# shichaoy/cube_slam

Hardware: NVIDIA H100
Metric: scored cuboid proposals/s (higher is better)
Workload: dtype f64

## Files before the change

### cube_slam_b200/_lib.py

```python
import ctypes as C
import os
import sys

import numpy as np

_HERE = os.path.dirname(os.path.abspath(__file__))
LIB_PATH = os.path.join(_HERE, "lib", "libcubeslam_b200.so")

CS_OK = 0
STATUS_NAMES = {0: "CS_OK", -1: "CS_ERR_INVALID_ARG", -2: "CS_ERR_CUDA", -3: "CS_ERR_CAPACITY",
                -4: "CS_ERR_NOT_PREPARED", -5: "CS_ERR_NCCL", -6: "CS_ERR_UNSUPPORTED"}


class CuboidParams(C.Structure):
    _fields_ = [
        ("consider_config_1", C.c_int32), ("consider_config_2", C.c_int32),
        ("whether_sample_cam_roll_pitch", C.c_int32), ("whether_sample_bbox_height", C.c_int32),
        ("max_cuboid_num", C.c_int32), ("reweight_edge_distance", C.c_int32),
        ("whether_normalize_two_errors", C.c_int32), ("top_sample_count_override", C.c_int32),
        ("nominal_skew_ratio", C.c_double), ("max_cut_skew", C.c_double),
        ("vp12_edge_angle_thre", C.c_double), ("vp3_edge_angle_thre", C.c_double),
        ("shorted_edge_thre", C.c_double), ("weight_vp_angle", C.c_double), ("weight_skew_error", C.c_double),
        ("pre_merge_dist_thre", C.c_double), ("pre_merge_angle_thre", C.c_double),
        ("edge_length_threshold", C.c_double), ("canny_low", C.c_double), ("canny_high", C.c_double),
# ... 85 lines not shown
    d.data = int(cai["data"][0])
    d.n_frames, d.height, d.width = shape[:3]
    d.channels = shape[3] if len(shape) == 4 else 1
    d.stride_frame, d.stride_row, d.stride_col = strides[:3]
    d.stride_channel = strides[3] if len(shape) == 4 else 0
    if isinstance(order, str):
        if order.lower() not in ORDERS:
            raise ValueError("order must be 'bgr' or 'rgb', got %r" % order)
        order = ORDERS[order.lower()]
    d.channel_order = int(order)
    d.stream = _stream_handle(frames, stream) or None
    return d


_lib = None

EXPORTS = [
    "cs_abi_version", "cs_create", "cs_destroy", "cs_last_error", "cs_default_cuboid_params",
    "cs_default_line_params", "cs_set_calibration", "cs_cam_pose", "cs_cuboid_measurement", "cs_cuboid_measurement_orb", "cs_detect_cuboids", "cs_detect_cuboids_batch",
    "cs_batch_upload", "cs_batch_upload_online", "cs_detect_frames_batch", "cs_batch_run", "cs_batch_run_async", "cs_batch_fetch", "cs_batch_stats_get",
    "cs_batch_device_records", "cs_stream", "cs_stage_ms", "cs_set_profiling", "cs_debug_roi",
    "cs_debug_candidates", "cs_detect_lines", "cs_detect_lines_batch", "cs_debug_lsd", "cs_debug_lsd_stats", "cs_debug_lsd_prof", "cs_debug_atan2", "cs_atan2_host", "cs_cuboid_draw_edges", "cs_debug_edlines", "cs_debug_stage_offsets", "cs_comm_unique_id", "cs_comm_init",
    "cs_allgather_topk", "cs_allgather_wait", "cs_fetch_gathered",
    "cs_keylines_from_lines", "cs_lbd_compute", "cs_lbd_compute_batch", "cs_detect_descrip_lines", "cs_detect_descrip_lines_batch",
    "cs_match_line_descrip", "cs_match_line_descrip_batch", "cs_lbd_debug_prepare", "cs_lbd_debug_keylines_edl", "cs_debug_last_set_pose",
]
DEVICE_FRAME_EXPORTS = ["cs_check_device_frames", "cs_batch_upload_device", "cs_batch_upload_online_device", "cs_detect_lines_batch_device"]
EXPORTS += DEVICE_FRAME_EXPORTS
MATCHER_EXPORTS = ["cs_knn_match_line_descrip", "cs_knn_match_line_descrip_batch", "cs_radius_match_line_descrip", "cs_radius_match_line_descrip_batch"]
EXPORTS += MATCHER_EXPORTS
COLLECTION_EXPORTS = ["cs_lbd_collection_create", "cs_lbd_collection_destroy", "cs_lbd_collection_add", "cs_lbd_collection_clear",
                      "cs_lbd_collection_size", "cs_lbd_collection_match", "cs_lbd_collection_knn_match", "cs_lbd_collection_radius_match"]
EXPORTS += COLLECTION_EXPORTS
LSD_DEBUG_EXPORTS = ["cs_debug_lsd_defb", "cs_debug_lsd_occupancy"]
EXPORTS += LSD_DEBUG_EXPORTS
NFA_DEBUG_EXPORTS = ["cs_debug_nfa"]
EXPORTS += NFA_DEBUG_EXPORTS
LBD_DEVICE_FRAME_EXPORTS = ["cs_detect_descrip_lines_batch_device", "cs_lbd_compute_batch_device"]
EXPORTS += LBD_DEVICE_FRAME_EXPORTS
OCTAVE_EXPORTS = ["cs_detect_raw_lines_octaves_batch", "cs_detect_descrip_lines_octaves_batch", "cs_detect_raw_lines_octaves_batch_device",
                  "cs_detect_descrip_lines_octaves_batch_device"]
EXPORTS += OCTAVE_EXPORTS
LBD_OCTAVE_EXPORTS = ["cs_lbd_compute_octaves_batch", "cs_lbd_compute_octaves_batch_device"]
EXPORTS += LBD_OCTAVE_EXPORTS
MIXED_EXPORTS = ["cs_detect_lines_batch_mixed", "cs_detect_raw_lines_octaves_batch_mixed"]
EXPORTS += MIXED_EXPORTS


def load():
    global _lib
    if _lib is not None:
        return _lib
    if not os.path.exists(LIB_PATH):
        raise OSError("%s is missing: build it with `python -m cube_slam_b200.build` (needs nvcc); "
                      "cube_slam_b200 has no CPU fallback" % LIB_PATH)
    L = C.CDLL(LIB_PATH)
    vp, i, d_p = C.c_void_p, C.c_int, C.POINTER(C.c_double)
    u8_p, i32_p, f_p = C.POINTER(C.c_uint8), C.POINTER(C.c_int32), C.POINTER(C.c_float)
    L.cs_abi_version.restype = i
    L.cs_create.restype = vp
    L.cs_create.argtypes = [i] * 6
    L.cs_destroy.argtypes = [vp]
    L.cs_destroy.restype = None
    L.cs_last_error.restype = C.c_char_p
    L.cs_last_error.argtypes = [vp]
    L.cs_default_cuboid_params.argtypes = [C.POINTER(CuboidParams)]
    L.cs_default_line_params.argtypes = [C.POINTER(LineParams)]
    L.cs_set_calibration.argtypes = [vp, d_p]
    L.cs_cam_pose.argtypes = [d_p, d_p, d_p, d_p]
    L.cs_cuboid_measurement.argtypes = [vp, d_p, d_p, d_p, d_p, d_p, d_p, d_p]
    L.cs_cuboid_measurement_orb.argtypes = [vp, d_p, C.c_double, d_p, d_p, d_p, d_p]
    L.cs_detect_cuboids.argtypes = [vp, u8_p, i, i, i, i, d_p, d_p, i, d_p, i, C.POINTER(CuboidParams), vp, i32_p]
    L.cs_detect_cuboids_batch.argtypes = [vp, vp, i, i, i, i, i, d_p, d_p, i32_p, d_p, i32_p, C.POINTER(CuboidParams), vp, i32_p]
    L.cs_batch_upload.argtypes = [vp, vp, i, i, i, i, i, d_p, d_p, i32_p, d_p, i32_p, C.POINTER(CuboidParams)]
    L.cs_batch_upload_online.argtypes = [vp, vp, i, i, i, i, i, d_p, d_p, i32_p, C.POINTER(LineParams), C.POINTER(CuboidParams)]
    L.cs_detect_frames_batch.argtypes = [vp, vp, i, i, i, i, i, d_p, d_p, i32_p, C.POINTER(LineParams), C.POINTER(CuboidParams), vp, i32_p]
    L.cs_batch_run.argtypes = [vp]
    L.cs_batch_run_async.argtypes = [vp]
    L.cs_batch_fetch.argtypes = [vp, vp, i32_p]
    L.cs_batch_stats_get.argtypes = [vp, C.POINTER(BatchStats)]
    L.cs_batch_device_records.argtypes = [vp, C.POINTER(vp), C.POINTER(C.c_size_t)]
    L.cs_stream.restype = vp
    L.cs_stream.argtypes = [vp]
    L.cs_stage_ms.argtypes = [vp, C.c_char_p, C.POINTER(C.c_float)]
    L.cs_set_profiling.argtypes = [vp, i]
    L.cs_debug_stage_offsets.argtypes = [vp, vp, f_p]
    L.cs_debug_roi.argtypes = [vp, i, i32_p, u8_p, f_p, i, d_p, i, i32_p, i32_p]
    L.cs_debug_candidates.argtypes = [vp, i, i32_p, u8_p, d_p, d_p, i]
    L.cs_detect_lines.argtypes = [vp, vp, i, i, i, i, C.POINTER(LineParams), f_p, i32_p]
    L.cs_detect_lines_batch.argtypes = [vp, vp, i, i, i, i, i, C.POINTER(LineParams), f_p, C.c_int32, i32_p]
    L.cs_debug_lsd.argtypes = [vp, i, i32_p, d_p, d_p, d_p, i32_p, i32_p, f_p, i32_p, i]
    L.cs_debug_lsd_stats.argtypes = [vp, i32_p, i32_p, i]
    L.cs_debug_lsd_prof.argtypes = [vp, C.POINTER(C.c_uint64), i]
    if hasattr(L, "cs_debug_lsd_defb"):
        L.cs_debug_lsd_defb.argtypes = [vp, i, C.POINTER(C.c_uint32), i32_p]
    if hasattr(L, "cs_debug_lsd_occupancy"):
        L.cs_debug_lsd_occupancy.argtypes = [vp, i32_p]
    L.cs_debug_atan2.argtypes = [vp, d_p, d_p, d_p, i]
    L.cs_atan2_host.argtypes = [C.c_double, C.c_double]
    L.cs_atan2_host.restype = C.c_double
    if hasattr(L, "cs_debug_nfa"):
        L.cs_debug_nfa.argtypes = [vp, i32_p, i32_p, d_p, C.c_double, i, d_p, i32_p, i]
    L.cs_cuboid_draw_edges.argtypes = [vp, i32_p]
    L.cs_debug_edlines.argtypes = [vp, i, u8_p, C.POINTER(C.c_int16), C.POINTER(C.c_int16), C.POINTER(C.c_int16), u8_p, i32_p, i32_p, u8_p, f_p, i32_p, i]
    L.cs_comm_unique_id.argtypes = [vp, C.c_char_p, u8_p]
    L.cs_comm_init.argtypes = [vp, C.c_char_p, u8_p, i, i]
    L.cs_allgather_topk.argtypes = [vp, i, C.POINTER(vp)]
    L.cs_allgather_wait.argtypes = [vp]
    L.cs_fetch_gathered.argtypes = [vp, vp, i]
    L.cs_keylines_from_lines.argtypes = [f_p, i, i, i, vp]
    L.cs_lbd_compute.argtypes = [vp, vp, i, i, i, i, vp, i, u8_p, f_p]
    L.cs_lbd_compute_batch.argtypes = [vp, vp, i, i, i, i, i, vp, i32_p, u8_p, f_p]
    L.cs_detect_descrip_lines.argtypes = [vp, vp, i, i, i, i, C.POINTER(LineParams), vp, u8_p, i32_p]
    L.cs_detect_descrip_lines_batch.argtypes = [vp, vp, i, i, i, i, i, C.POINTER(LineParams), vp, u8_p, C.c_int32, i32_p]
    L.cs_match_line_descrip.argtypes = [vp, u8_p, i, u8_p, i, C.c_float, vp, i32_p]
    L.cs_match_line_descrip_batch.argtypes = [vp, u8_p, i32_p, u8_p, i32_p, i, C.c_float, vp, i32_p]
    i64_p = C.POINTER(C.c_int64)
    if all(hasattr(L, n) for n in MATCHER_EXPORTS):
        L.cs_knn_match_line_descrip.argtypes = [vp, u8_p, i, u8_p, i, i, u8_p, vp, i32_p]
        L.cs_knn_match_line_descrip_batch.argtypes = [vp, u8_p, i32_p, u8_p, i32_p, i, i, u8_p, vp, i32_p]
        L.cs_radius_match_line_descrip.argtypes = [vp, u8_p, i, u8_p, i, C.c_float, u8_p, vp, C.c_int64, i64_p]
        L.cs_radius_match_line_descrip_batch.argtypes = [vp, u8_p, i32_p, u8_p, i32_p, i, C.c_float, u8_p, vp, C.c_int64, i64_p]
    if all(hasattr(L, n) for n in COLLECTION_EXPORTS):
        L.cs_lbd_collection_create.restype = vp
        L.cs_lbd_collection_create.argtypes = [vp]
        L.cs_lbd_collection_destroy.restype = None
        L.cs_lbd_collection_destroy.argtypes = [vp]
        L.cs_lbd_collection_add.argtypes = [vp, u8_p, i32_p, i]
        L.cs_lbd_collection_clear.argtypes = [vp]
        L.cs_lbd_collection_size.argtypes = [vp, i32_p, i64_p]
# ... 43 lines not shown
```

### cube_slam_b200/csrc/cs_lsd.cu

```cuda
#include <cuda_runtime.h>
#include <float.h>
#include <math.h>
#include <stdint.h>

#include <algorithm>
#include <cmath>
#include <cstring>
#include <vector>

#include "cs_internal.h"
#include "cs_nfa.cuh"
#include "cs_tma.cuh"

#define LSD_PI 3.1415926535897932384626433832795
#define LSD_NOTDEF (-1024.0)
#define LSD_DEG2RAD (LSD_PI / 180)
#define LSD_3_2_PI ((3 * LSD_PI) / 2)
#define LSD_2PI (2 * LSD_PI)
#define LSD_LN10 2.30258509299404568402
#define LSD_NBINS 1024
#define LSD_CHUNK_ROWS 8
#define LSD_SCALE 0.8

#define LSD_CAND_CAP 2048
// ... 946 lines not shown
        ((sy < pre_boundary_thre) && (ey < pre_boundary_thre)) || ((sy > img_h - pre_boundary_thre) && (ey > img_h - pre_boundary_thre)))
        return false;
    const double ddx = (double)(e[0] - e[2]), ddy = (double)(e[1] - e[3]);
    const float line_length = (float)sqrt(ddx * ddx + ddy * ddy);
    if (!(line_length > line_length_thres)) return false;
    o[0] = sx;
    o[1] = sy;
    o[2] = ex;
    o[3] = ey;
    return true;
}

struct LsdGrowArgs {
    int W, H, img_w, img_h;
    uint4 *pix;
    const float *angf;
    const double *modgrad;
    int32_t *arena;
    int arena_cap;
    double LOG_NT;
    int min_reg_size;
    double prec, p, scale;
    float line_length_thres;
    float *raw;
    int32_t *n_raw;
    float *out;
    int32_t *n_out;
    int cap;
    LsdRect *cand;
    int32_t *n_cand;
    int cand_cap;
    int32_t *cand_line;
    struct LsdCandState *cand_state;
    int32_t *err;
    const double *lgam;
    uint32_t *ubits;
    const uint32_t *defb;
    const LsdGeom *geom;
};

template <bool kProf, bool kMixed>
__global__ void __launch_bounds__(32, 21) k_lsd_grow_seq(LsdGrowArgs A)
{
    const int f = blockIdx.x, lane = threadIdx.x;
    LsdGeom G = {};
    if constexpr (kMixed) G = A.geom[f];
    const int fW = kMixed ? G.W : A.W, fH = kMixed ? G.H : A.H;
    const size_t npx = (size_t)fW * fH;
    const size_t px0 = kMixed ? (size_t)G.px_off : f * npx;
    LsdFrame F;
    LSD_PROF_T0();
    F.W = fW;
    F.H = fH;
    F.pix = A.pix + px0;
    F.angf = A.angf + px0;
    F.modgrad = A.modgrad + px0;
    F.LOG_NT = kMixed ? G.LOG_NT : A.LOG_NT;
    const int WW = (fW + 31) >> 5, n_words = WW * fH;
    const size_t w0f = kMixed ? (size_t)G.bit_off : (size_t)f * n_words;
    F.ubits = A.ubits + w0f;
    F.WW = WW;
    F.span = nullptr;
    F.lgam = A.lgam;
    F.wmagic = ((1ull << 40) + (unsigned long long)fW - 1) / (unsigned long long)fW;
    for (int i = lane; i < n_words; i += 32) F.ubits[i] = 0u;
    __syncwarp();
// ... 23 lines not shown
            }
            if (!nz) break;
            const int j = __ffs(nz) - 1;
            const int b = __ffs(__shfl_sync(0xffffffffu, s, j)) - 1;
            const int s_addr = __shfl_sync(0xffffffffu, w_addr, j) + b;
            int n_all = 0, has_rect = 0;
            LsdRect rec;
            const long long c0 = kProf ? clock64() : 0ll;
            lsd_grow_candidate<kProf>(F, R, s_addr, min_reg_size, A.prec, A.p, n_all, has_rect, rec);
            if (kProf) {
                in_cand += clock64() - c0;
                if (lane == 0) {
                    atomicAdd(&g_lsd_prof[4], 1ull);
                    if (n_all > LSD_SEQ_SCAP) atomicAdd(&g_lsd_prof[8], 1ull);
                }
            }
            if (kProf) handoff_t0 = clock64();
            __syncwarp();
            u = wi < n_words ? __ldcg(F.ubits + wi) : 0u;
            u_next = wi + 32 < n_words ? __ldcg(F.ubits + wi + 32) : 0u;
            s = d & ~u & (lane > j ? 0xffffffffu : lane == j ? 0xfffffffeu << b : 0u);
            if (!has_rect) continue;
            const long long st0 = kProf ? clock64() : 0ll;
            if (lane == 0 && n_cand < A.cand_cap) A.cand[(size_t)f * A.cand_cap + n_cand] = rec;
            n_cand++;
            if (kProf) {
                const long long dt = clock64() - st0;
                if (lane == 0) atomicAdd(&g_lsd_prof[10], (unsigned long long)dt);
                handoff_t0 += dt;
            }
        }
    }
    if (kProf && lane == 0) atomicAdd(&g_lsd_prof[3], (unsigned long long)(clock64() - scan_t0 - in_cand));
    if (lane == 0) {
        A.n_cand[f] = n_cand;
        if (n_cand > A.cand_cap) {
            atomicOr(A.err, 4);
            atomicMax(A.err + 1, n_cand);
            A.err[2] = A.cand_cap;
        }
    }
    LSD_PROF_ADD(6);
}

#define LSD_VAL_CTAS 64

struct LsdCandState {
    double log_nfa;
    int32_t status;
    int32_t n;
    int32_t tot[5], alg[5];
};

__device__ int lsd_improve_variants(const LsdRect &rec, int round, LsdRect *cand)
{
    const double delta = 0.5, delta_2 = delta / 2.0;
    LsdRect r = rec;
    if (round == 0) {
        cand[0] = r;
        return 1;
    }
    if (round == 1) {
        for (int n = 0; n < 5; ++n) {
            r.p /= 2;
            r.prec = r.p * LSD_PI;
            cand[n] = r;
        }
        return 5;
    }
    const int phase = round - 2;
    int m = 0;
    for (int n = 0; n < 5; ++n)
        if ((r.width - delta) >= 0.5) {
            if (phase == 0)
                r.width -= delta;
            else if (phase == 1) {
                r.x1 += -r.dy * delta_2;
                r.y1 += r.dx * delta_2;
                r.x2 += -r.dy * delta_2;
                r.y2 += r.dx * delta_2;
                r.width -= delta;
            } else if (phase == 2) {
                r.x1 -= -r.dy * delta_2;
                r.y1 -= r.dx * delta_2;
                r.x2 -= -r.dy * delta_2;
                r.y2 -= r.dx * delta_2;
                r.width -= delta;
            } else {
                r.p /= 2;
                r.prec = r.p * LSD_PI;
            }
            cand[m++] = r;
        }
    return m;
}

template <bool kMixed>
__global__ void __launch_bounds__(128, 5) k_lsd_val_count(LsdGrowArgs A, int round)
{
    const int f = kMixed ? (int)(blockIdx.x / LSD_VAL_CTAS) : (int)blockIdx.y, lane = threadIdx.x & 31;
    const int bx = kMixed ? (int)(blockIdx.x % LSD_VAL_CTAS) : (int)blockIdx.x, gx = kMixed ? LSD_VAL_CTAS : (int)gridDim.x;
    LsdFrame F;
    if constexpr (kMixed) {
        const LsdGeom &G = A.geom[f];
        F.W = G.W;
        F.H = G.H;
        F.angf = A.angf + G.px_off;
        F.LOG_NT = G.LOG_NT;
    } else {
        const size_t npx = (size_t)A.W * A.H;
        F.W = A.W;
        F.H = A.H;
        F.angf = A.angf + f * npx;
        F.LOG_NT = A.LOG_NT;
    }
    F.pix = nullptr;
    F.modgrad = nullptr;
    F.ubits = nullptr;
    __shared__ LsdSpan s_span[4][5];
    F.span = s_span[threadIdx.x >> 5];
    F.lgam = A.lgam;
    F.wmagic = 0;
    const int n = min(A.n_cand[f], A.cand_cap);
    const int wpb = blockDim.x >> 5;
    for (int c = bx * wpb + (threadIdx.x >> 5); c < n; c += gx * wpb) {
        LsdCandState *S = A.cand_state + (size_t)f * A.cand_cap + c;
        if (round > 0 && S->status != 0) continue;
        const LsdRect rec = A.cand[(size_t)f * A.cand_cap + c];
        LsdRect cv[5];
        const int m = lsd_improve_variants(rec, round, cv);
        int tot[5] = {0, 0, 0, 0, 0}, alg[5] = {0, 0, 0, 0, 0};
        if (m == 1)
            lsd_rect_count(F, cv[0], tot[0], alg[0]);
        else if (m > 1)
            lsd_rect_count_multi(F, cv, m, round == 1 || round == 5, tot, alg);
        if (lane == 0) {
            S->n = m;
            for (int t = 0; t < 5; t++) {
                S->tot[t] = tot[t];
                S->alg[t] = alg[t];
            }
        }
    }
}

template <bool kMixed>
__global__ void __launch_bounds__(128, 5) k_lsd_val_nfa(LsdGrowArgs A, int round)
{
    const int f = kMixed ? (int)(blockIdx.x / LSD_VAL_CTAS) : (int)blockIdx.y, lane = threadIdx.x & 31;
    const int bx = kMixed ? (int)(blockIdx.x % LSD_VAL_CTAS) : (int)blockIdx.x, gx = kMixed ? LSD_VAL_CTAS : (int)gridDim.x;
    const double LOG_NT = kMixed ? A.geom[f].LOG_NT : A.LOG_NT;
    const int n = min(A.n_cand[f], A.cand_cap);
    const int wpb = blockDim.x >> 5;
    for (int c = bx * wpb + (threadIdx.x >> 5); c < n; c += gx * wpb) {
        LsdCandState *S = A.cand_state + (size_t)f * A.cand_cap + c;
        if (round > 0 && S->status != 0) continue;
        LsdRect rec = A.cand[(size_t)f * A.cand_cap + c];
        LsdRect cv[5];
        const int m = lsd_improve_variants(rec, round, cv);
        double log_nfa = round == 0 ? 0.0 : S->log_nfa;
        bool changed = false;
        for (int t = 0; t < m; t++) {
            const double v = cs_nfa_warp(A.lgam, S->tot[t], S->alg[t], cv[t].p, LOG_NT, true);
            if (round == 0 || v > log_nfa) {
                log_nfa = v;
                rec = cv[t];
                changed = round > 0;
            }
        }
        const bool done = round == 5 || log_nfa > 0.0;
        __syncwarp();
        if (lane == 0) {
            if (done) {
                int32_t *o = A.cand_line + ((size_t)f * A.cand_cap + c) * 5;
                const bool ok = log_nfa > 0.0;
                o[0] = ok ? 1 : 0;
                o[1] = __float_as_int((float)((rec.x1 + 0.5) / A.scale));
                o[2] = __float_as_int((float)((rec.y1 + 0.5) / A.scale));
                o[3] = __float_as_int((float)((rec.x2 + 0.5) / A.scale));
                o[4] = __float_as_int((float)((rec.y2 + 0.5) / A.scale));
                S->status = 1;
            } else {
                if (changed) A.cand[(size_t)f * A.cand_cap + c] = rec;
                S->log_nfa = log_nfa;
                S->status = 0;
            }
        }
    }
}

#define LSD_LAUNCHES_PER_RUN 15

template <bool kMixed>
__global__ void __launch_bounds__(256) k_lsd_emit(LsdGrowArgs A)
{
    __shared__ int s_warp_cnt[8], s_base_raw, s_base_out;
    const int f = blockIdx.x, tid = threadIdx.x, lane = tid & 31, wid = tid >> 5;
    const unsigned FULL = 0xffffffffu;
    const int n = min(A.n_cand[f], A.cand_cap);
    float *raw = A.raw + (size_t)f * A.cap * 4;
    float *out = A.out + (size_t)f * A.cap * 4;
    if (tid == 0) {
        s_base_raw = 0;
        s_base_out = 0;
    }
    __syncthreads();
    for (int b = 0; b < n; b += 256) {
        const int i = b + tid;
        bool has = false, kept = false;
        float ln[4], fo[4];
        if (i < n) {
            const int32_t *o = A.cand_line + ((size_t)f * A.cand_cap + i) * 5;
            if (o[0]) {
                has = true;
                for (int k = 0; k < 4; k++) ln[k] = __int_as_float(o[1 + k]);
                kept = lsd_keyline_filter(ln, kMixed ? A.geom[f].w : A.img_w, kMixed ? A.geom[f].h : A.img_h, A.line_length_thres, fo);
            }
        }
// ... 11 lines not shown
                for (int k = 0; k < 4; k++) raw[4 * slot + k] = ln[k];
        }
        if (kept) {
            const int slot = pre_o + __popc(mk & ((1u << lane) - 1u));
            if (slot < A.cap)
                for (int k = 0; k < 4; k++) out[4 * slot + k] = fo[k];
        }
        __syncthreads();
        if (tid == 0) {
            int tr = 0, to = 0;
            for (int k = 0; k < 8; k++) {
                tr += s_warp_cnt[k] & 0xffff;
                to += s_warp_cnt[k] >> 16;
            }
            s_base_raw += tr;
            s_base_out += to;
        }
        __syncthreads();
    }
    if (tid == 0) {
        const bool overflow = A.n_cand[f] > A.cand_cap;
        A.n_raw[f] = overflow ? A.cap + 1 : s_base_raw;
        A.n_out[f] = overflow ? A.cap + 1 : s_base_out;
    }
}

struct Buf {
    void *p = nullptr;
    size_t cap = 0;
};

struct LsdState {
    CsLineHead head;
    Buf img, modgrad, angf, pix, defb, arena, raw, nraw, out, nout, lgam, ubits, cand, ncand, candline, candstate, err, geom;
    bool lgam_filled = false;
    bool last_mixed = false;
    int last_frames = 0, last_W = 0, last_H = 0, cap = 0;
    const uint8_t *last_img = nullptr;
    int last_w = 0, last_h = 0, last_stride = 0, last_channels = 0;
    int cand_cap = LSD_CAND_CAP;
};

int ensure(cs_ctx *c, Buf &b, size_t bytes)
{
    if (bytes <= b.cap) return CS_OK;
    if (b.p) cudaFree(b.p);
    b.p = nullptr;
    b.cap = 0;
    const size_t want = bytes + bytes / 16 + 256;
    if (cudaMalloc(&b.p, want) != cudaSuccess) return cs_ctx_fail(c, CS_ERR_CUDA, "cudaMalloc(%zu) failed in the line detector", want);
    b.cap = want;
    return CS_OK;
}

inline int grid_for(int64_t n) { return (int)std::min<int64_t>((n + 255) / 256, CS_SM_COUNT * 32); }

void lsd_front(cs_ctx *c, const uint8_t *d_img, int n_frames, int w, int h, int stride, int channels, int W, int H, double rho, double *modgrad,
               float *angf, uint4 *pix, uint32_t *defb, double *scaled, int32_t *d_err)
{
    cudaStream_t st = cs_ctx_stream(c);
    const dim3 g_tile((W + LSF_TW - 1) / LSF_TW, (H + LSF_TH - 1) / LSF_TH, n_frames);
    const double inv_scale = 1. / LSD_SCALE;
    CUtensorMap tm;
    memset(&tm, 0, sizeof tm);
    if (scaled)
        k_lsd_front<false, true, false><<<g_tile, 256, 0, st>>>(tm, d_img, w, h, stride, channels, W, H, inv_scale, rho, modgrad, angf, pix, defb, scaled,
                                                                d_err, nullptr, 0);
    else if (cs_ctx_use_tma(c) && channels == 3 && stride == 3 * w &&
             cs_make_tmap_bytes(&tm, d_img, 3 * (int64_t)w, (int64_t)n_frames * h, stride, LSF_BOXW, LSF_GH))
        k_lsd_front<true, false, false><<<g_tile, 256, 0, st>>>(tm, d_img, w, h, stride, channels, W, H, inv_scale, rho, modgrad, angf, pix, defb, nullptr,
                                                                d_err, nullptr, 0);
    else
        k_lsd_front<false, false, false><<<g_tile, 256, 0, st>>>(tm, d_img, w, h, stride, channels, W, H, inv_scale, rho, modgrad, angf, pix, defb,
                                                                 nullptr, d_err, nullptr, 0);
}

const double LSD_ANG_TH = 22.5, LSD_QUANT = 2.0;
inline double lsd_prec() { return LSD_PI * LSD_ANG_TH / 180; }
inline double lsd_p() { return LSD_ANG_TH / 180; }
inline double lsd_log_nt(int W, int H) { return 5 * (std::log10((double)W) + std::log10((double)H)) / 2 + std::log10(11.0); }
inline int lsd_min_reg_size(double LOG_NT) { return (int)(-LOG_NT / std::log10(lsd_p())); }
inline int lsd_arena_cap(int W, int H) { return (int)(((size_t)W * H * 2 + 64 + 3) & ~(size_t)3); }

int lsd_buffers(cs_ctx *c, LsdState &S, int n_frames, size_t spx, size_t bit_words, size_t arena_ints, int cap)
{
    int rc;
    if ((rc = ensure(c, S.modgrad, spx * 8)) || (rc = ensure(c, S.angf, spx * 4)) || (rc = ensure(c, S.pix, spx * 16)) || (rc = ensure(c, S.defb, bit_words * 4)) ||
        (rc = ensure(c, S.arena, arena_ints * 4)) ||
        (rc = ensure(c, S.raw, (size_t)n_frames * cap * 16)) || (rc = ensure(c, S.nraw, (size_t)n_frames * 4)) ||
        (rc = ensure(c, S.out, (size_t)n_frames * cap * 16)) || (rc = ensure(c, S.nout, (size_t)n_frames * 4)) ||
        (rc = ensure(c, S.lgam, (size_t)CS_LGAMMA_TABLE * 8)) || (rc = ensure(c, S.ubits, bit_words * 4)) ||
        (rc = ensure(c, S.cand, (size_t)n_frames * S.cand_cap * sizeof(LsdRect))) || (rc = ensure(c, S.ncand, (size_t)n_frames * 4)) ||
        (rc = ensure(c, S.candline, (size_t)n_frames * S.cand_cap * 20)) || (rc = ensure(c, S.candstate, (size_t)n_frames * S.cand_cap * sizeof(LsdCandState))) || (rc = ensure(c, S.err, 16)))
        return rc;
    if (!S.lgam_filled) {
        std::vector<double> t(CS_LGAMMA_TABLE, 0.0);
        for (int i = 1; i < CS_LGAMMA_TABLE; i++) t[i] = cs_lgamma_host((double)i);
        if (cudaMemcpyAsync(S.lgam.p, t.data(), t.size() * 8, cudaMemcpyHostToDevice, cs_ctx_stream(c)) != cudaSuccess ||
            cudaStreamSynchronize(cs_ctx_stream(c)) != cudaSuccess)
            return cs_ctx_fail(c, CS_ERR_CUDA, "upload of the log_gamma table failed");
        S.lgam_filled = true;
    }
    S.head.d_err = (int32_t *)S.err.p;
    cudaMemsetAsync(S.err.p, 0, 16, cs_ctx_stream(c));
    return CS_OK;
}

LsdGrowArgs lsd_args(const LsdState &S, int cap, float line_length_thres)
{
    LsdGrowArgs A;
    memset(&A, 0, sizeof A);
    A.pix = (uint4 *)S.pix.p;
    A.angf = (const float *)S.angf.p;
    A.modgrad = (const double *)S.modgrad.p;
    A.arena = (int32_t *)S.arena.p;
    A.prec = lsd_prec();
    A.p = lsd_p();
    A.scale = LSD_SCALE;
    A.line_length_thres = line_length_thres;
    A.raw = (float *)S.raw.p;
    A.n_raw = (int32_t *)S.nraw.p;
    A.out = (float *)S.out.p;
    A.n_out = (int32_t *)S.nout.p;
    A.cap = cap;
    A.lgam = (const double *)S.lgam.p;
    A.ubits = (uint32_t *)S.ubits.p;
    A.defb = (const uint32_t *)S.defb.p;
    A.cand = (LsdRect *)S.cand.p;
    A.n_cand = (int32_t *)S.ncand.p;
    A.cand_cap = S.cand_cap;
    A.cand_line = (int32_t *)S.candline.p;
    A.cand_state = (LsdCandState *)S.candstate.p;
    A.err = (int32_t *)S.err.p;
    return A;
}

template <bool kMixed>
int lsd_seed_loop(cs_ctx *c, const LsdGrowArgs &A, int n_frames)
{
    cudaStream_t st = cs_ctx_stream(c);
    const size_t smem = LSD_SEQ_SMEM;
    if (cs_ctx_profiling(c))
        k_lsd_grow_seq<true, kMixed><<<n_frames, 32, smem, st>>>(A);
    else
        k_lsd_grow_seq<false, kMixed><<<n_frames, 32, smem, st>>>(A);
    const dim3 g_val = kMixed ? dim3(LSD_VAL_CTAS * n_frames) : dim3(LSD_VAL_CTAS, n_frames);
    for (int round = 0; round < 6; round++) {
        k_lsd_val_count<kMixed><<<g_val, 128, 0, st>>>(A, round);
        k_lsd_val_nfa<kMixed><<<g_val, 128, 0, st>>>(A, round);
    }
    k_lsd_emit<kMixed><<<n_frames, 256, 0, st>>>(A);
    cs_ctx_count_launches(c, LSD_LAUNCHES_PER_RUN);
    if (cudaGetLastError() != cudaSuccess) return cs_ctx_fail(c, CS_ERR_CUDA, "LSD kernel launch failed: %s", cudaGetErrorString(cudaGetLastError()));
    return CS_OK;
}

int lsd_run(cs_ctx *c, const uint8_t *imgs, bool imgs_on_device, int n_frames, int w, int h, int stride, int channels, float line_length_thres,
            int cap, LsdState &S)
{
    cudaStream_t st = cs_ctx_stream(c);
    const int W = (int)std::lrint(w * LSD_SCALE), H = (int)std::lrint(h * LSD_SCALE);
    if (W < 2 || H < 2) return cs_ctx_fail(c, CS_ERR_INVALID_ARG, "image too small for LSD");
    const size_t spx = (size_t)n_frames * W * H;
    const size_t bit_words = (size_t)n_frames * ((W + 31) / 32) * H;
    const int arena_cap = lsd_arena_cap(W, H);
    int rc;
    const uint8_t *d_img = imgs;
    if (!imgs_on_device) {
        if ((rc = ensure(c, S.img, (size_t)n_frames * h * stride))) return rc;
        if (cudaMemcpyAsync(S.img.p, imgs, (size_t)n_frames * h * stride, cudaMemcpyHostToDevice, st) != cudaSuccess)
            return cs_ctx_fail(c, CS_ERR_CUDA, "H2D copy of frames failed");
        d_img = (const uint8_t *)S.img.p;
    }
    if ((rc = lsd_buffers(c, S, n_frames, spx, bit_words, (size_t)n_frames * arena_cap, cap))) return rc;
    const double rho = LSD_QUANT / std::sin(lsd_prec());
    const double LOG_NT = lsd_log_nt(W, H);
    lsd_front(c, d_img, n_frames, w, h, stride, channels, W, H, rho, (double *)S.modgrad.p, (float *)S.angf.p, (uint4 *)S.pix.p, (uint32_t *)S.defb.p,
              nullptr, (int32_t *)S.err.p);
    LsdGrowArgs A = lsd_args(S, cap, line_length_thres);
    A.W = W;
    A.H = H;
    A.img_w = w;
    A.img_h = h;
    A.arena_cap = arena_cap;
    A.LOG_NT = LOG_NT;
    A.min_reg_size = lsd_min_reg_size(LOG_NT);
    if ((rc = lsd_seed_loop<false>(c, A, n_frames))) return rc;
    S.last_mixed = false;
    S.last_frames = n_frames;
    S.last_W = W;
    S.last_H = H;
    S.cap = cap;
    S.last_img = d_img;
    S.last_w = w;
    S.last_h = h;
    S.last_stride = stride;
    S.last_channels = channels;
    return CS_OK;
}

int lsd_run_mixed(cs_ctx *c, const uint8_t *d_img, const cs_frame_view *views, int n_frames, float line_length_thres, int cap, LsdState &S)
{
    cudaStream_t st = cs_ctx_stream(c);
    static_assert((int64_t)CS_LSD_MAX_MIXED_FRAMES * LSD_VAL_CTAS <= INT32_MAX, "the validation grid of a mixed run");
    if (n_frames > CS_LSD_MAX_MIXED_FRAMES)
        return cs_ctx_fail(c, CS_ERR_CAPACITY, "%d frames in one LSD batch: at most %d", n_frames, CS_LSD_MAX_MIXED_FRAMES);
    std::vector<LsdGeom> g((size_t)n_frames);
    size_t spx = 0, bit_words = 0, arena_ints = 0;
    int64_t tiles = 0;
    for (int f = 0; f < n_frames; f++) {
        const cs_frame_view &v = views[f];
        LsdGeom &G = g[(size_t)f];
        memset(&G, 0, sizeof G);
        G.W = (int)std::lrint(v.width * LSD_SCALE);
        G.H = (int)std::lrint(v.height * LSD_SCALE);
        if (G.W < 2 || G.H < 2) return cs_ctx_fail(c, CS_ERR_INVALID_ARG, "frame %d: a %d x %d image is too small for LSD", f, v.width, v.height);
        G.img_off = v.offset;
        G.w = v.width;
        G.h = v.height;
        G.stride = v.stride;
        G.channels = v.channels;
        G.LOG_NT = lsd_log_nt(G.W, G.H);
        G.min_reg_size = lsd_min_reg_size(G.LOG_NT);
        G.tiles_x = (G.W + LSF_TW - 1) / LSF_TW;
        G.tile0 = (int)tiles;
        tiles += (int64_t)G.tiles_x * ((G.H + LSF_TH - 1) / LSF_TH);
        G.px_off = (int64_t)spx;
        spx += (size_t)G.W * G.H;
        G.bit_off = (int64_t)bit_words;
        bit_words += (size_t)((G.W + 31) / 32) * G.H;
        G.arena_off = (int64_t)arena_ints;
        arena_ints += (size_t)lsd_arena_cap(G.W, G.H);
    }
    if (tiles > INT32_MAX) return cs_ctx_fail(c, CS_ERR_CAPACITY, "%lld front-end tiles in one batch: more than a grid holds", (long long)tiles);
    int rc;
    if ((rc = ensure(c, S.geom, g.size() * sizeof(LsdGeom))) || (rc = lsd_buffers(c, S, n_frames, spx, bit_words, arena_ints, cap))) return rc;
    if (cudaMemcpyAsync(S.geom.p, g.data(), g.size() * sizeof(LsdGeom), cudaMemcpyHostToDevice, st) != cudaSuccess)
        return cs_ctx_fail(c, CS_ERR_CUDA, "upload of the LSD frame table failed");
    const LsdGeom *d_geom = (const LsdGeom *)S.geom.p;
    CUtensorMap tm;
    memset(&tm, 0, sizeof tm);
    k_lsd_front<false, false, true><<<(unsigned)tiles, 256, 0, st>>>(tm, d_img, 0, 0, 0, 0, 0, 0, 1. / LSD_SCALE, LSD_QUANT / std::sin(lsd_prec()),
                                                                     (double *)S.modgrad.p, (float *)S.angf.p, (uint4 *)S.pix.p, (uint32_t *)S.defb.p, nullptr,
                                                                     (int32_t *)S.err.p, d_geom, n_frames);
    LsdGrowArgs A = lsd_args(S, cap, line_length_thres);
    A.geom = d_geom;
    if ((rc = lsd_seed_loop<true>(c, A, n_frames))) return rc;
    S.last_mixed = true;
    S.last_frames = n_frames;
    S.cap = cap;
    return CS_OK;
}

LsdState *state_of(cs_ctx *c)
{
    void **slot = cs_ctx_lsd_slot(c);
    if (!*slot) *slot = new LsdState();
    return (LsdState *)*slot;
}

bool lsd_grow_candidates(LsdState &S, const int32_t err[4])
{
    if (!(err[0] & 4) || err[1] <= S.cand_cap) return false;
    S.cand_cap = (err[1] + 255) & ~255;
    return true;
}

}

int cs_lsd_run_device(cs_ctx *c, const uint8_t *d_imgs, int n_frames, int w, int h, int stride, int channels, float line_length_thres, int cap,
                      const float **d_lines, const int32_t **d_counts)
{
    LsdState *S = state_of(c);
    const int rc = lsd_run(c, d_imgs, true, n_frames, w, h, stride, channels, line_length_thres, cap, *S);
    if (rc) return rc;
    *d_lines = (const float *)S->out.p;
    *d_counts = (const int32_t *)S->nout.p;
    return CS_OK;
}

// ... 319 lines not shown
    if (reset) {
        const unsigned long long z[16] = {0};
        cudaMemcpyToSymbol(g_lsd_prof, z, 128);
    }
    return cudaGetLastError() == cudaSuccess ? CS_OK : cs_ctx_fail(c, CS_ERR_CUDA, "debug copy failed");
}

int cs_debug_lsd_occupancy(cs_ctx *c, int32_t *out14)
{
    if (!c || !out14) return CS_ERR_INVALID_ARG;
    cudaSetDevice(cs_ctx_device(c));
    struct {
        const void *fn;
        int threads, dyn_smem;
    } const k[2] = {{(const void *)k_lsd_grow_seq<false, false>, 32, LSD_SEQ_SMEM}, {(const void *)k_lsd_front<true, false, false>, 256, 0}};
    for (int i = 0; i < 2; i++) {
        cudaFuncAttributes a;
        int per_sm = 0;
        if (cudaFuncGetAttributes(&a, k[i].fn) != cudaSuccess ||
            cudaOccupancyMaxActiveBlocksPerMultiprocessor(&per_sm, k[i].fn, k[i].threads, k[i].dyn_smem) != cudaSuccess)
            return cs_ctx_fail(c, CS_ERR_CUDA, "LSD kernel attribute query failed: %s", cudaGetErrorString(cudaGetLastError()));
        int32_t *o = out14 + 7 * i;
        o[0] = a.numRegs;
        o[1] = (int32_t)a.localSizeBytes;
        o[2] = (int32_t)a.sharedSizeBytes;
        o[3] = k[i].dyn_smem;
        o[4] = k[i].threads;
        o[5] = per_sm;
        o[6] = a.preferredShmemCarveout;
    }
    return CS_OK;
}

int cs_debug_lsd_stats(cs_ctx *c, int32_t *stats4, int32_t *redo, int n_frames)
{
    if (!c) return CS_ERR_INVALID_ARG;
    LsdState *S = state_of(c);
    if (n_frames > S->last_frames) return cs_ctx_fail(c, CS_ERR_INVALID_ARG, "more frames than the last run held");
    if (stats4) memset(stats4, 0, (size_t)n_frames * 16);
    if (redo)
        for (int f = 0; f < n_frames; f++) redo[f] = 1;
    return CS_OK;
}
}
```

### include/cube_slam_b200.h

```cpp
#ifndef CUBE_SLAM_B200_H
#define CUBE_SLAM_B200_H

#include <stddef.h>
#include <stdint.h>

#ifdef __cplusplus
extern "C" {
#endif

#define CS_ABI_VERSION 1

typedef enum cs_status {
    CS_OK = 0,
    CS_ERR_INVALID_ARG = -1,
    CS_ERR_CUDA = -2,
    CS_ERR_CAPACITY = -3,
    CS_ERR_NOT_PREPARED = -4,
    CS_ERR_NCCL = -5,
    CS_ERR_UNSUPPORTED = -6
} cs_status;

typedef struct cs_ctx cs_ctx;

typedef struct cs_cuboid_params {
// ... 130 lines not shown
int cs_batch_device_records(cs_ctx *ctx, void **dev_ptr, size_t *n_bytes);
void *cs_stream(cs_ctx *ctx);
int cs_stage_ms(cs_ctx *ctx, const char *stage, float *ms);
int cs_set_profiling(cs_ctx *ctx, int enable);
int cs_debug_last_set_pose(const uint8_t *valid, const double *dist_err, const double *angle_err, int n_cand, int n_pose, int32_t *pose_out);

int cs_debug_stage_offsets(cs_ctx *ctx, cs_ctx *ref, float offsets_ms[9]);

int cs_debug_roi(cs_ctx *ctx, int job, int32_t roi_xywh[4], uint8_t *canny, float *dist, int cap_px,
                 double *merged_lines, int cap_lines, int32_t *n_lines_roi, int32_t *n_lines_merged);
int cs_debug_candidates(cs_ctx *ctx, int job, int32_t *n_candidates, uint8_t *valid, double *dist_err,
                        double *angle_err, int cap);

int cs_detect_lines(cs_ctx *ctx, const uint8_t *img, int width, int height, int stride, int channels,
                    const cs_line_params *params, float *lines_xyxy, int32_t *n_inout);
int cs_detect_lines_batch(cs_ctx *ctx, const uint8_t *imgs, int n_frames, int width, int height, int stride,
                          int channels, const cs_line_params *params, float *lines_xyxy, int32_t max_lines_per_frame,
                          int32_t *n_lines );

typedef struct cs_frame_view {
    int64_t offset;
    int32_t width, height, stride, channels;
} cs_frame_view;

int cs_detect_lines_batch_mixed(cs_ctx *ctx, const uint8_t *imgs, const cs_frame_view *views, int n_frames, const cs_line_params *params,
                                float *lines_xyxy, int32_t max_lines_per_frame, int32_t *n_lines );

int cs_debug_lsd(cs_ctx *ctx, int frame, int32_t scaled_wh[2], double *scaled, double *modgrad, double *angles, int32_t *list,
                 int32_t *list_len, float *raw_lines, int32_t *n_raw, int cap_raw);
int cs_debug_lsd_stats(cs_ctx *ctx, int32_t *stats4, int32_t *redo, int n_frames);
int cs_debug_lsd_prof(cs_ctx *ctx, uint64_t *out16, int reset);
int cs_debug_lsd_occupancy(cs_ctx *ctx, int32_t *out14);
int cs_debug_lsd_defb(cs_ctx *ctx, int frame, uint32_t *bits, int32_t *words_per_row);
int cs_debug_edlines(cs_ctx *ctx, int frame, uint8_t *blur, int16_t *dx, int16_t *dy, int16_t *g, uint8_t *dir, int32_t *anchors,
                     int32_t *n_anchors, uint8_t *edge, float *raw_lines, int32_t *n_raw, int cap_raw);

typedef struct cs_keyline {
    float start_x, start_y, end_x, end_y;
    float angle;
    float line_length;
    float response;
    float size;
    int32_t num_pixels;
    int32_t class_id;
} cs_keyline;
typedef struct cs_dmatch {
    int32_t query_idx, train_idx, img_idx;
    float distance;
} cs_dmatch;

int cs_keylines_from_lines(const float *lines_xyxy, int n, int width, int height, cs_keyline *out);

int cs_lbd_compute(cs_ctx *ctx, const uint8_t *img, int width, int height, int stride, int channels, const cs_keyline *keylines, int n,
                   uint8_t *desc32, float *desc72);
int cs_lbd_compute_batch(cs_ctx *ctx, const uint8_t *imgs, int n_frames, int width, int height, int stride, int channels,
                         const cs_keyline *keylines, const int32_t *keyline_offsets , uint8_t *desc32, float *desc72);

int cs_detect_descrip_lines(cs_ctx *ctx, const uint8_t *img, int width, int height, int stride, int channels, const cs_line_params *params,
                            cs_keyline *keylines, uint8_t *desc32, int32_t *n_inout);
int cs_detect_descrip_lines_batch(cs_ctx *ctx, const uint8_t *imgs, int n_frames, int width, int height, int stride, int channels,
                                  const cs_line_params *params, cs_keyline *keylines, uint8_t *desc32, int32_t max_lines_per_frame,
                                  int32_t *n_lines );

typedef struct cs_keyline_octave {
    cs_keyline kl;
    float s_oct_x, s_oct_y, e_oct_x, e_oct_y;
// ... 74 lines not shown
```

Baseline: 9.139 million.

## Compact LSD validation rounds into worklists of unresolved candidates

The seed kernel now appends each frame's candidates to a global (frame, index) worklist, and each NFA validation round pushes candidates that are still unresolved into the next round's list. Later rounds launch a grid sized from pixel count over just the surviving entries, instead of a fixed per-frame grid that scans every candidate and skips finished ones by reading a status flag. This aims to cut wasted warps and load imbalance in validation rounds one through five. The cost is global atomics for list appends, extra buffers, and a debug export for list lengths.

```diff
diff --git a/cube_slam_b200/_lib.py b/cube_slam_b200/_lib.py
--- a/cube_slam_b200/_lib.py
+++ b/cube_slam_b200/_lib.py
@@ -141,7 +141,7 @@
 COLLECTION_EXPORTS = ["cs_lbd_collection_create", "cs_lbd_collection_destroy", "cs_lbd_collection_add", "cs_lbd_collection_clear",
                       "cs_lbd_collection_size", "cs_lbd_collection_match", "cs_lbd_collection_knn_match", "cs_lbd_collection_radius_match"]
 EXPORTS += COLLECTION_EXPORTS
-LSD_DEBUG_EXPORTS = ["cs_debug_lsd_defb", "cs_debug_lsd_occupancy"]
+LSD_DEBUG_EXPORTS = ["cs_debug_lsd_defb", "cs_debug_lsd_occupancy", "cs_debug_lsd_val_lists"]
 EXPORTS += LSD_DEBUG_EXPORTS
 NFA_DEBUG_EXPORTS = ["cs_debug_nfa"]
 EXPORTS += NFA_DEBUG_EXPORTS
@@ -205,6 +205,8 @@
         L.cs_debug_lsd_defb.argtypes = [vp, i, C.POINTER(C.c_uint32), i32_p]
     if hasattr(L, "cs_debug_lsd_occupancy"):
         L.cs_debug_lsd_occupancy.argtypes = [vp, i32_p]
+    if hasattr(L, "cs_debug_lsd_val_lists"):
+        L.cs_debug_lsd_val_lists.argtypes = [vp, i32_p]
     L.cs_debug_atan2.argtypes = [vp, d_p, d_p, d_p, i]
     L.cs_atan2_host.argtypes = [C.c_double, C.c_double]
     L.cs_atan2_host.restype = C.c_double
diff --git a/cube_slam_b200/csrc/cs_lsd.cu b/cube_slam_b200/csrc/cs_lsd.cu
--- a/cube_slam_b200/csrc/cs_lsd.cu
+++ b/cube_slam_b200/csrc/cs_lsd.cu
@@ -1002,6 +1002,8 @@
     int cand_cap;
     int32_t *cand_line;
     struct LsdCandState *cand_state;
+    int2 *vlist[2];
+    int32_t *vcount;
     int32_t *err;
     const double *lgam;
     uint32_t *ubits;
@@ -1091,6 +1093,8 @@
         }
     }
     if (kProf && lane == 0) atomicAdd(&g_lsd_prof[3], (unsigned long long)(clock64() - scan_t0 - in_cand));
+    const int n_val = min(n_cand, A.cand_cap);
+    int base = 0;
     if (lane == 0) {
         A.n_cand[f] = n_cand;
         if (n_cand > A.cand_cap) {
@@ -1098,15 +1102,20 @@
             atomicMax(A.err + 1, n_cand);
             A.err[2] = A.cand_cap;
         }
-    }
+        if (n_val) base = atomicAdd(A.vcount, n_val);
+    }
+    base = __shfl_sync(0xffffffffu, base, 0);
+    for (int i = lane; i < n_val; i += 32) A.vlist[0][base + i] = make_int2(f, i);
     LSD_PROF_ADD(6);
 }
 
-#define LSD_VAL_CTAS 64
+#define LSD_VAL_THREADS 128
+#define LSD_VAL_CTAS0 64
+#define LSD_VAL_LATE_PX 24576
+#define LSD_VAL_ROUNDS 6
 
 struct LsdCandState {
     double log_nfa;
-    int32_t status;
     int32_t n;
     int32_t tot[5], alg[5];
 };
@@ -1155,36 +1164,35 @@
 }
 
 template <bool kMixed>
-__global__ void __launch_bounds__(128, 5) k_lsd_val_count(LsdGrowArgs A, int round)
-{
-    const int f = kMixed ? (int)(blockIdx.x / LSD_VAL_CTAS) : (int)blockIdx.y, lane = threadIdx.x & 31;
-    const int bx = kMixed ? (int)(blockIdx.x % LSD_VAL_CTAS) : (int)blockIdx.x, gx = kMixed ? LSD_VAL_CTAS : (int)gridDim.x;
+__global__ void __launch_bounds__(LSD_VAL_THREADS, 5) k_lsd_val_count(LsdGrowArgs A, int round)
+{
+    const int lane = threadIdx.x & 31, wpb = LSD_VAL_THREADS / 32;
     LsdFrame F;
-    if constexpr (kMixed) {
-        const LsdGeom &G = A.geom[f];
-        F.W = G.W;
-        F.H = G.H;
-        F.angf = A.angf + G.px_off;
-        F.LOG_NT = G.LOG_NT;
-    } else {
-        const size_t npx = (size_t)A.W * A.H;
-        F.W = A.W;
-        F.H = A.H;
-        F.angf = A.angf + f * npx;
-        F.LOG_NT = A.LOG_NT;
-    }
     F.pix = nullptr;
     F.modgrad = nullptr;
     F.ubits = nullptr;
-    __shared__ LsdSpan s_span[4][5];
+    __shared__ LsdSpan s_span[LSD_VAL_THREADS / 32][5];
     F.span = s_span[threadIdx.x >> 5];
     F.lgam = A.lgam;
     F.wmagic = 0;
-    const int n = min(A.n_cand[f], A.cand_cap);
-    const int wpb = blockDim.x >> 5;
-    for (int c = bx * wpb + (threadIdx.x >> 5); c < n; c += gx * wpb) {
+    const int n = A.vcount[round];
+    const int2 *list = A.vlist[round & 1];
+    for (int i = blockIdx.x * wpb + (threadIdx.x >> 5); i < n; i += gridDim.x * wpb) {
+        const int2 e = list[i];
+        const int f = e.x, c = e.y;
+        if constexpr (kMixed) {
+            const LsdGeom &G = A.geom[f];
+            F.W = G.W;
+            F.H = G.H;
+            F.angf = A.angf + G.px_off;
+            F.LOG_NT = G.LOG_NT;
+        } else {
+            F.W = A.W;
+            F.H = A.H;
+            F.angf = A.angf + (size_t)f * A.W * A.H;
+            F.LOG_NT = A.LOG_NT;
+        }
         LsdCandState *S = A.cand_state + (size_t)f * A.cand_cap + c;
-        if (round > 0 && S->status != 0) continue;
         const LsdRect rec = A.cand[(size_t)f * A.cand_cap + c];
         LsdRect cv[5];
         const int m = lsd_improve_variants(rec, round, cv);
@@ -1204,16 +1212,16 @@
 }
 
 template <bool kMixed>
-__global__ void __launch_bounds__(128, 5) k_lsd_val_nfa(LsdGrowArgs A, int round)
-{
-    const int f = kMixed ? (int)(blockIdx.x / LSD_VAL_CTAS) : (int)blockIdx.y, lane = threadIdx.x & 31;
-    const int bx = kMixed ? (int)(blockIdx.x % LSD_VAL_CTAS) : (int)blockIdx.x, gx = kMixed ? LSD_VAL_CTAS : (int)gridDim.x;
-    const double LOG_NT = kMixed ? A.geom[f].LOG_NT : A.LOG_NT;
-    const int n = min(A.n_cand[f], A.cand_cap);
-    const int wpb = blockDim.x >> 5;
-    for (int c = bx * wpb + (threadIdx.x >> 5); c < n; c += gx * wpb) {
+__global__ void __launch_bounds__(LSD_VAL_THREADS, 5) k_lsd_val_nfa(LsdGrowArgs A, int round)
+{
+    const int lane = threadIdx.x & 31, wpb = LSD_VAL_THREADS / 32;
+    const int n = A.vcount[round];
+    const int2 *list = A.vlist[round & 1];
+    for (int i = blockIdx.x * wpb + (threadIdx.x >> 5); i < n; i += gridDim.x * wpb) {
+        const int2 e = list[i];
+        const int f = e.x, c = e.y;
+        const double LOG_NT = kMixed ? A.geom[f].LOG_NT : A.LOG_NT;
         LsdCandState *S = A.cand_state + (size_t)f * A.cand_cap + c;
-        if (round > 0 && S->status != 0) continue;
         LsdRect rec = A.cand[(size_t)f * A.cand_cap + c];
         LsdRect cv[5];
         const int m = lsd_improve_variants(rec, round, cv);
@@ -1238,11 +1246,10 @@
                 o[2] = __float_as_int((float)((rec.y1 + 0.5) / A.scale));
                 o[3] = __float_as_int((float)((rec.x2 + 0.5) / A.scale));
                 o[4] = __float_as_int((float)((rec.y2 + 0.5) / A.scale));
-                S->status = 1;
             } else {
                 if (changed) A.cand[(size_t)f * A.cand_cap + c] = rec;
                 S->log_nfa = log_nfa;
-                S->status = 0;
+                A.vlist[(round + 1) & 1][atomicAdd(A.vcount + round + 1, 1)] = e;
             }
         }
     }
@@ -1320,13 +1327,14 @@
 
 struct LsdState {
     CsLineHead head;
-    Buf img, modgrad, angf, pix, defb, arena, raw, nraw, out, nout, lgam, ubits, cand, ncand, candline, candstate, err, geom;
+    Buf img, modgrad, angf, pix, defb, arena, raw, nraw, out, nout, lgam, ubits, cand, ncand, candline, candstate, vlist, vcount, err, geom;
     bool lgam_filled = false;
     bool last_mixed = false;
     int last_frames = 0, last_W = 0, last_H = 0, cap = 0;
     const uint8_t *last_img = nullptr;
     int last_w = 0, last_h = 0, last_stride = 0, last_channels = 0;
     int cand_cap = LSD_CAND_CAP;
+    size_t vlist_cap = 0;
 };
 
 int ensure(cs_ctx *c, Buf &b, size_t bytes)
@@ -1379,7 +1387,8 @@
         (rc = ensure(c, S.out, (size_t)n_frames * cap * 16)) || (rc = ensure(c, S.nout, (size_t)n_frames * 4)) ||
         (rc = ensure(c, S.lgam, (size_t)CS_LGAMMA_TABLE * 8)) || (rc = ensure(c, S.ubits, bit_words * 4)) ||
         (rc = ensure(c, S.cand, (size_t)n_frames * S.cand_cap * sizeof(LsdRect))) || (rc = ensure(c, S.ncand, (size_t)n_frames * 4)) ||
-        (rc = ensure(c, S.candline, (size_t)n_frames * S.cand_cap * 20)) || (rc = ensure(c, S.candstate, (size_t)n_frames * S.cand_cap * sizeof(LsdCandState))) || (rc = ensure(c, S.err, 16)))
+        (rc = ensure(c, S.candline, (size_t)n_frames * S.cand_cap * 20)) || (rc = ensure(c, S.candstate, (size_t)n_frames * S.cand_cap * sizeof(LsdCandState))) ||
+        (rc = ensure(c, S.vlist, 2 * (size_t)n_frames * S.cand_cap * sizeof(int2))) || (rc = ensure(c, S.vcount, LSD_VAL_ROUNDS * 4)) || (rc = ensure(c, S.err, 16)))
         return rc;
     if (!S.lgam_filled) {
         std::vector<double> t(CS_LGAMMA_TABLE, 0.0);
@@ -1391,6 +1400,8 @@
     }
     S.head.d_err = (int32_t *)S.err.p;
     cudaMemsetAsync(S.err.p, 0, 16, cs_ctx_stream(c));
+    cudaMemsetAsync(S.vcount.p, 0, LSD_VAL_ROUNDS * 4, cs_ctx_stream(c));
+    S.vlist_cap = n_frames * (size_t)S.cand_cap;
     return CS_OK;
 }
 
@@ -1419,12 +1430,15 @@
     A.cand_cap = S.cand_cap;
     A.cand_line = (int32_t *)S.candline.p;
     A.cand_state = (LsdCandState *)S.candstate.p;
+    A.vlist[0] = (int2 *)S.vlist.p;
+    A.vlist[1] = A.vlist[0] + S.vlist_cap;
+    A.vcount = (int32_t *)S.vcount.p;
     A.err = (int32_t *)S.err.p;
     return A;
 }
 
 template <bool kMixed>
-int lsd_seed_loop(cs_ctx *c, const LsdGrowArgs &A, int n_frames)
+int lsd_seed_loop(cs_ctx *c, const LsdGrowArgs &A, int n_frames, size_t spx)
 {
     cudaStream_t st = cs_ctx_stream(c);
     const size_t smem = LSD_SEQ_SMEM;
@@ -1432,10 +1446,11 @@
         k_lsd_grow_seq<true, kMixed><<<n_frames, 32, smem, st>>>(A);
     else
         k_lsd_grow_seq<false, kMixed><<<n_frames, 32, smem, st>>>(A);
-    const dim3 g_val = kMixed ? dim3(LSD_VAL_CTAS * n_frames) : dim3(LSD_VAL_CTAS, n_frames);
-    for (int round = 0; round < 6; round++) {
-        k_lsd_val_count<kMixed><<<g_val, 128, 0, st>>>(A, round);
-        k_lsd_val_nfa<kMixed><<<g_val, 128, 0, st>>>(A, round);
+    const int g_first = (int)std::min<int64_t>((int64_t)n_frames * LSD_VAL_CTAS0, INT32_MAX);
+    const int g_late = (int)std::min<size_t>(spx / LSD_VAL_LATE_PX + 1, INT32_MAX);
+    for (int round = 0; round < LSD_VAL_ROUNDS; round++) {
+        k_lsd_val_count<kMixed><<<round ? g_late : g_first, LSD_VAL_THREADS, 0, st>>>(A, round);
+        k_lsd_val_nfa<kMixed><<<round ? g_late : g_first, LSD_VAL_THREADS, 0, st>>>(A, round);
     }
     k_lsd_emit<kMixed><<<n_frames, 256, 0, st>>>(A);
     cs_ctx_count_launches(c, LSD_LAUNCHES_PER_RUN);
@@ -1473,7 +1488,7 @@
     A.arena_cap = arena_cap;
     A.LOG_NT = LOG_NT;
     A.min_reg_size = lsd_min_reg_size(LOG_NT);
-    if ((rc = lsd_seed_loop<false>(c, A, n_frames))) return rc;
+    if ((rc = lsd_seed_loop<false>(c, A, n_frames, spx))) return rc;
     S.last_mixed = false;
     S.last_frames = n_frames;
     S.last_W = W;
@@ -1490,7 +1505,6 @@
 int lsd_run_mixed(cs_ctx *c, const uint8_t *d_img, const cs_frame_view *views, int n_frames, float line_length_thres, int cap, LsdState &S)
 {
     cudaStream_t st = cs_ctx_stream(c);
-    static_assert((int64_t)CS_LSD_MAX_MIXED_FRAMES * LSD_VAL_CTAS <= INT32_MAX, "the validation grid of a mixed run");
     if (n_frames > CS_LSD_MAX_MIXED_FRAMES)
         return cs_ctx_fail(c, CS_ERR_CAPACITY, "%d frames in one LSD batch: at most %d", n_frames, CS_LSD_MAX_MIXED_FRAMES);
     std::vector<LsdGeom> g((size_t)n_frames);
@@ -1533,7 +1547,7 @@
                                                                      (int32_t *)S.err.p, d_geom, n_frames);
     LsdGrowArgs A = lsd_args(S, cap, line_length_thres);
     A.geom = d_geom;
-    if ((rc = lsd_seed_loop<true>(c, A, n_frames))) return rc;
+    if ((rc = lsd_seed_loop<true>(c, A, n_frames, spx))) return rc;
     S.last_mixed = true;
     S.last_frames = n_frames;
     S.cap = cap;
@@ -1919,6 +1933,18 @@
     return CS_OK;
 }
 
+int cs_debug_lsd_val_lists(cs_ctx *c, int32_t *rounds6)
+{
+    if (!c || !rounds6) return CS_ERR_INVALID_ARG;
+    cudaSetDevice(cs_ctx_device(c));
+    LsdState *S = state_of(c);
+    if (!S->vcount.p) return cs_ctx_fail(c, CS_ERR_INVALID_ARG, "no LSD run on this context yet");
+    if (cudaMemcpyAsync(rounds6, S->vcount.p, LSD_VAL_ROUNDS * 4, cudaMemcpyDeviceToHost, cs_ctx_stream(c)) != cudaSuccess ||
+        cudaStreamSynchronize(cs_ctx_stream(c)) != cudaSuccess)
+        return cs_ctx_fail(c, CS_ERR_CUDA, "validation list lengths copy failed: %s", cudaGetErrorString(cudaGetLastError()));
+    return CS_OK;
+}
+
 int cs_debug_lsd_stats(cs_ctx *c, int32_t *stats4, int32_t *redo, int n_frames)
 {
     if (!c) return CS_ERR_INVALID_ARG;
diff --git a/include/cube_slam_b200.h b/include/cube_slam_b200.h
--- a/include/cube_slam_b200.h
+++ b/include/cube_slam_b200.h
@@ -186,6 +186,7 @@
 int cs_debug_lsd_prof(cs_ctx *ctx, uint64_t *out16, int reset);
 int cs_debug_lsd_occupancy(cs_ctx *ctx, int32_t *out14);
 int cs_debug_lsd_defb(cs_ctx *ctx, int frame, uint32_t *bits, int32_t *words_per_row);
+int cs_debug_lsd_val_lists(cs_ctx *ctx, int32_t *rounds6);
 int cs_debug_edlines(cs_ctx *ctx, int frame, uint8_t *blur, int16_t *dx, int16_t *dy, int16_t *g, uint8_t *dir, int32_t *anchors,
                      int32_t *n_anchors, uint8_t *edge, float *raw_lines, int32_t *n_raw, int cap_raw);
 
```

Result: faster. 9.324 million (median of 6 runs) (+2.0%).
